# African-Robotics-Unit/AcinoSet

Hardware: AMD Instinct MI355X
Metric: FTE frames/sec (residual+Jac+LM step), 6-cam x 20-joint (higher is better)
Workload: dtype f64

## Files before the change

acinoset_amd/csrc/chunk.hip:

```cpp
#include "chunk.hpp"

#include <algorithm>
#include <cstdlib>
#include <type_traits>

#include "bcr_dev.hpp"
#include "trio80.hpp"

namespace acino {

void ChunkPlan::build(int nodes_total, int chunk_nodes, bool pin_l, bool pin_r) {
  n_nodes = nodes_total;
  m = n_chunks = n_sep = 0;
  node0 = pin_l ? 1 : 0;
  pin_right = pin_r ? 1 : 0;
  const int nodes = nodes_total - node0;
  if (chunk_nodes < 0 || nodes < 1) return;
  int mm = chunk_nodes;
  if (mm == 0) {
    mm = (nodes + 255) / 256;
    mm = std::max(4, std::min(mm, 512));
  }
  mm = std::max(2, mm);
  m = mm;
  n_chunks = (nodes + mm - 1) / mm;
  if (pin_r && n_chunks > 1 && nodes - (n_chunks - 1) * mm == 1) --n_chunks;
  n_sep = n_chunks - 1 + node0 + pin_right;
}

__device__ __forceinline__ void tile_store(double* M, int ib, int jb, const d4& a, int li, int lk) {
#pragma unroll
  for (int rr = 0; rr < 4; ++rr) M[(ib * 16 + lk + 4 * rr) * LD + jb * 16 + li] = a[rr];
}

constexpr int SW_VEC = 18 * NP + 2 * BS + 8 + 8 + 3 * NP + 64;
static constexpr size_t kSweepLds = (3 * MAT + SW_VEC) * sizeof(double);

__device__ __forceinline__ int opaque(int x) {
  asm volatile("" : "+v"(x));
  return x;
}

__device__ __forceinline__ unsigned opaque_u(unsigned x) {
  asm volatile("" : "+v"(x));
  return x;
}
struct BuildSlot {
  int pr, pc, base, e;
  bool own, dg;
  static __device__ __forceinline__ BuildSlot unpack(unsigned w) {
    BuildSlot s;
    s.pr = w & 31;
    s.pc = (w >> 5) & 31;
    s.own = (w >> 10) & 1;
    s.dg = (w >> 11) & 1;
    s.base = (w >> 12) & 2047;
    s.e = w >> 23;
    return s;
  }
};
static_assert((NP - 1) * LD + NP - 1 < 2048 && 13 * NP <= 512 && NP <= 32, "BuildSlot's bit fields");

constexpr int SW_T = 512;
template <int NQ>
__device__ __forceinline__ void syrk_mask_n(d4 (&acc)[NQ], bool load) {
#pragma unroll
  for (int q = 0; q < NQ; ++q)
#pragma unroll
    for (int rr = 0; rr < 4; ++rr) acc[q][rr] = load ? acc[q][rr] : 0.0;
}
constexpr int SP_STEPS = 4 * NT - 1;
__device__ __forceinline__ void spike_gf(const double* G, const double (&bF)[NT][4], d4 (&acc)[NT], int li, int lk) {
  double a[3][NT];
  const double* gb = G + lk * LD + li;
  auto fetch = [&](int buf, int step) {
#pragma unroll
    for (int ib = 0; ib < NT; ++ib) a[buf][ib] = gb[(4 * step) * LD + ib * 16];
  };
#pragma unroll
  for (int ib = 0; ib < NT; ++ib) acc[ib] = d4{0, 0, 0, 0};
  fetch(0, 0);
  fetch(1, 1);
#pragma unroll
  for (int step = 0; step < SP_STEPS; ++step) {
    if (step + 2 < SP_STEPS) fetch((step + 2) % 3, step + 2);
    __builtin_amdgcn_sched_barrier(0);
#pragma unroll
    for (int ib = 0; ib < NT; ++ib) acc[ib] = mfma(a[step % 3][ib], bF[step >> 2][step & 3], acc[ib]);
    __builtin_amdgcn_sched_barrier(0);
  }
}
template <int NQ>
__device__ __forceinline__ void spike_ftt(d4 (&acc)[NQ], const double* Yf, const d4 (&T)[NT], const int (&as)[NQ], int li, int lk) {
  constexpr int DEPTH = NQ >= 3 ? 2 : (NQ == 2 ? 3 : 6);
  const double* p = Yf + lk * LD + li;
  double a[DEPTH + 1][NQ];
#pragma unroll
  for (int d = 0; d < DEPTH; ++d)
#pragma unroll
    for (int q = 0; q < NQ; ++q) a[d][q] = p[(4 * d) * LD + as[q] * 16];
#pragma unroll
  for (int st = 0; st < SP_STEPS; ++st) {
    if (st + DEPTH < SP_STEPS) {
#pragma unroll
      for (int q = 0; q < NQ; ++q) a[(st + DEPTH) % (DEPTH + 1)][q] = p[(4 * (st + DEPTH)) * LD + as[q] * 16];
    }
    __builtin_amdgcn_sched_barrier(0);
#pragma unroll
    for (int q = 0; q < NQ; ++q) acc[q] = mfma(-a[st % (DEPTH + 1)][q], T[st >> 2][st & 3], acc[q]);
    __builtin_amdgcn_sched_barrier(0);
  }
}
template <int NQ>
struct AlTiles {
  d4 acc[NQ];
  int as[NQ], j;
  double* Ag;
  __device__ __forceinline__ double* at(int q, int rr, int li, int lk) const {
    return as[q] >= j ? Ag + (size_t)(as[q] * 16 + 4 * rr + lk) * BS + j * 16 + li
                      : Ag + (size_t)(j * 16 + li) * BS + as[q] * 16 + 4 * rr + lk;
  }
  __device__ __forceinline__ void fetch(int li, int lk) {
#pragma unroll
    for (int q = 0; q < NQ; ++q)
#pragma unroll
      for (int rr = 0; rr < 4; ++rr) acc[q][rr] = *at(q, rr, li, lk);
  }
  __device__ __forceinline__ void run(bool load, const double* Yf, const d4 (&T)[NT], int li, int lk) {
    syrk_mask_n<NQ>(acc, load);
    spike_ftt<NQ>(acc, Yf, T, as, li, lk);
#pragma unroll
    for (int q = 0; q < NQ; ++q)
#pragma unroll
      for (int rr = 0; rr < 4; ++rr) *at(q, rr, li, lk) = acc[q][rr];
  }
};
__device__ __forceinline__ int role8(int wave) { return (0x75236410u >> (4 * wave)) & 15; }
constexpr int ctri_i(int t) { return (t >= 1) + (t >= 3) + (t >= 6) + (t >= 10); }
template <int T>
struct GramTile {
  static constexpr int ib = ctri_i(T), jb = T - ib * (ib + 1) / 2, ns = 4 * (NT - ib);
};
template <int T>
__device__ __forceinline__ void gram_fetch(const double* X, int li, int lk, double (&a)[GramTile<T>::ns], double (&b)[GramTile<T>::ns]) {
  const double* pa = X + (GramTile<T>::ib * 16 + li) * LD + GramTile<T>::ib * 16 + lk;
  const double* pb = X + (GramTile<T>::jb * 16 + li) * LD + GramTile<T>::ib * 16 + lk;
#pragma unroll
  for (int s = 0; s < GramTile<T>::ns; ++s) {
    a[s] = pa[4 * s];
    b[s] = pb[4 * s];
  }
}
template <int T>
__device__ __forceinline__ void gram_tile(double* Xg, int li, int lk, const double (&a)[GramTile<T>::ns], const double (&b)[GramTile<T>::ns]) {
  constexpr int ib = GramTile<T>::ib, jb = GramTile<T>::jb;
  d4 g = {0, 0, 0, 0};
#pragma unroll
  for (int s = 0; s < GramTile<T>::ns; ++s) g = mfma(a[s], b[s], g);
#pragma unroll
  for (int rr = 0; rr < 4; ++rr) {
    Xg[(ib * 16 + lk + 4 * rr) * LD + jb * 16 + li] = g[rr];
    if (ib != jb) Xg[(jb * 16 + li) * LD + ib * 16 + lk + 4 * rr] = g[rr];
  }
}
template <int T0, int... REST>
__device__ __forceinline__ void gram_chain(const double* Xf, double* Xg, int li, int lk, const double (&a)[GramTile<T0>::ns],
                                           const double (&b)[GramTile<T0>::ns]) {
  if constexpr (sizeof...(REST) > 0) {
    constexpr int rest[] = {REST...};
    double an[GramTile<rest[0]>::ns], bn[GramTile<rest[0]>::ns];
    gram_fetch<rest[0]>(Xf, li, lk, an, bn);
    __builtin_amdgcn_sched_barrier(0);
    gram_tile<T0>(Xg, li, lk, a, b);
    __builtin_amdgcn_sched_barrier(0);
    gram_chain<REST...>(Xf, Xg, li, lk, an, bn);
  } else {
    gram_tile<T0>(Xg, li, lk, a, b);
  }
}
template <int T0, int... REST>
__device__ __forceinline__ void gram_fixed(const double* Xf, double* Xg, int* done, int li, int lk, int lane) {
  double a[GramTile<T0>::ns], b[GramTile<T0>::ns];
  gram_fetch<T0>(Xf, li, lk, a, b);
  gram_chain<T0, REST...>(Xf, Xg, li, lk, a, b);
  asm volatile("" ::: "memory");
  if (lane == 0) __hip_atomic_fetch_add(done, 1 + (int)sizeof...(REST), __ATOMIC_RELAXED, __HIP_MEMORY_SCOPE_WORKGROUP);
  asm volatile("" ::: "memory");
}

struct SpikeArgs {
  const double* Xg;
  double* Y;
  double* Ag;
  const double* cRk;
  const double* bvn;
  double* zk;
  int *c_gfdone, *c_fready, *c_bv, *tdone;
  int *g_open, *g_done;
  const double* Xf;
  int k, n_s;
  bool hasL, has_next;
  long long* stamps;
};
template <int ROLE>
__device__ __forceinline__ void spike_node(const SpikeArgs& A, int& tsb, int ln) {
  constexpr bool two = ROLE == 5;
  constexpr int j0 = ROLE == 4 ? 1 : (ROLE == 5 ? 2 : (ROLE == 6 ? 3 : 4));
  constexpr int NA = ROLE == 4 ? 3 : (ROLE == 5 ? 2 : (ROLE == 6 ? 5 : 4));
  const int li = ln & 15, lk = ln >> 4;
  double* const Y = A.Y;
  auto stamp = [&](int i) { if (A.stamps && ln == 0) A.stamps[i] = (long long)wall_clock64(); };
  AlTiles<NA> al;
  AlTiles<1> al0;
  al.Ag = A.Ag;
  al.j = j0;
  if (ROLE == 4) { al.as[0] = 1; al.as[1] = 0; al.as[2 % NA] = 2; }
  if (ROLE == 5) { al.as[0] = 2; al.as[1] = 0; }
  if (ROLE == 6) { al.as[0] = 3; al.as[1] = 0; al.as[2 % NA] = 1; al.as[3 % NA] = 2; al.as[4 % NA] = 4; }
  if (ROLE == 7) { al.as[0] = 4; al.as[1] = 0; al.as[2 % NA] = 1; al.as[3 % NA] = 2; }
  al0.Ag = A.Ag;
  al0.j = 0;
  al0.as[0] = 0;
  if (A.hasL) {
    al.fetch(li, lk);
    if (two) al0.fetch(li, lk);
  }
  if (ROLE >= 6) {
    double* const Xg = const_cast<double*>(A.Xg);
    lds_wait(A.g_open, A.k + 1);
    if (ROLE == 6) gram_fixed<2, 13>(A.Xf, Xg, A.g_done, li, lk, ln);
    else if (A.hasL) gram_fixed<5, 9, 14>(A.Xf, Xg, A.g_done, li, lk, ln);
    else gram_fixed<2, 5, 9, 13, 14>(A.Xf, Xg, A.g_done, li, lk, ln);
  }
  lds_wait(A.g_done, 15 * (A.k + 1));
  stamp(16 + 4 * (ROLE - 4));
  d4 T0[NT], T1[NT];
  {
    double bF[NT][4];
    const double* yb = Y + lk * LD + j0 * 16 + li;
#pragma unroll
    for (int kb = 0; kb < NT; ++kb)
#pragma unroll
      for (int s = 0; s < 4; ++s) bF[kb][s] = (4 * kb + s < SP_STEPS) ? yb[(kb * 16 + 4 * s) * LD] : 0.0;
    spike_gf(A.Xg, bF, T0, li, lk);
  }
  if (two) {
    double bF[NT][4];
    const double* yb = Y + lk * LD + li;
#pragma unroll
    for (int kb = 0; kb < NT; ++kb)
#pragma unroll
      for (int s = 0; s < 4; ++s) bF[kb][s] = (4 * kb + s < SP_STEPS) ? yb[(kb * 16 + 4 * s) * LD] : 0.0;
    spike_gf(A.Xg, bF, T1, li, lk);
  }
  lds_signal(A.c_gfdone, ln);
  stamp(17 + 4 * (ROLE - 4));
  if (A.hasL) {
    lds_wait(A.c_fready, A.n_s * A.k);
    al.run(A.k > 0, Y, T0, li, lk);
    if (two) al0.run(A.k > 0, Y, T1, li, lk);
  }
  stamp(18 + 4 * (ROLE - 4));
  if (A.hasL) {
    if (ROLE != 5) lds_signal(A.tdone + (ROLE == 4 ? 0 : (ROLE == 6 ? 1 : 2)), ln);
    if (ROLE == 7 || ROLE == 4 || ROLE == 5) lds_wait(A.tdone + 1, A.k + 1);
    if (ROLE == 4 || ROLE == 5) lds_wait(A.tdone + 2, A.k + 1);
    if (ROLE == 5) lds_wait(A.tdone + 0, A.k + 1);
  }
  (void)tsb;
#pragma unroll
  for (int ib = 0; ib < NT; ++ib) tile_store(Y, ib, j0, T0[ib], li, lk);
  if (two) {
#pragma unroll
    for (int ib = 0; ib < NT; ++ib) tile_store(Y, ib, 0, T1[ib], li, lk);
  }
  if (ROLE == 7) {
    A.zk[ln] = Y[ln * LD + (BS - 1)];
    if (ln < 16) A.zk[64 + ln] = Y[(64 + ln) * LD + (BS - 1)];
  }
  if (A.has_next) {
    lds_wait(A.c_bv, A.k + 1);
    const double* const cRk = A.cRk;
    const double* const bvn = A.bvn;
    const int p = ln % NP, cg = ln / NP;
#pragma unroll
    for (int h = 0; h < (two ? 2 : 1); ++h) {
      const int c_lo = 16 * (h ? 0 : j0);
      if (cg < 2) {
        const double e00 = cRk[(0 * 3 + 0) * NP + p], e01 = cRk[(0 * 3 + 1) * NP + p], e02 = cRk[(0 * 3 + 2) * NP + p];
        const double e11 = cRk[(1 * 3 + 1) * NP + p], e12 = cRk[(1 * 3 + 2) * NP + p], e22 = cRk[(2 * 3 + 2) * NP + p];
        const double b0 = bvn[p], b1 = bvn[NP + p], b2 = bvn[2 * NP + p];
        double fv[8][3];
#pragma unroll
        for (int q = 0; q < 8; ++q) {
          const int cc = c_lo + cg + 2 * q;
          fv[q][0] = Y[p * LD + cc];
          fv[q][1] = Y[(NP + p) * LD + cc];
          fv[q][2] = Y[(2 * NP + p) * LD + cc];
        }
#pragma unroll
        for (int q = 0; q < 8; ++q) {
          const int cc = c_lo + cg + 2 * q;
          const double f0 = fv[q][0], f1 = fv[q][1], f2 = fv[q][2];
          double o0 = -(e00 * f0 + e01 * f1 + e02 * f2), o1 = -(e11 * f1 + e12 * f2), o2 = -(e22 * f2);
          if (cc == BS - 1) {
            o0 += b0;
            o1 += b1;
            o2 += b2;
          }
          Y[p * LD + cc] = o0;
          Y[(NP + p) * LD + cc] = o1;
          Y[(2 * NP + p) * LD + cc] = o2;
        }
      }
      if (ln < 16)
        for (int r = 3 * NP; r < BS; ++r) Y[r * LD + c_lo + ln] = 0.0;
    }
  }
  lds_signal(A.c_fready, ln);
  stamp(19 + 4 * (ROLE - 4));
}


__global__ void __launch_bounds__(SW_T)
k_chunk_sweep(BcrChain ch, SepView sp, const FteConst* __restrict__ cst, int* numeric_err, const int* __restrict__ status,
                int m, int n_chunks, int node0, int pin_right) {
  extern __shared__ __attribute__((aligned(16))) char smem_raw[];
  if (status && *status != 0) return;
  double* const Xf = reinterpret_cast<double*>(smem_raw);
  double* const Xg = Xf + MAT;
  double* const Y = Xg + MAT;
  double* const cL = Y + MAT;
  double* const cR0 = cL + 9 * NP;
  double* const bvb = cR0 + 9 * NP;
  double* const red = bvb + 2 * BS;
  int* const sync = reinterpret_cast<int*>(red + 8);
  int* const cB = sync + 5;
  int* const tdone = sync + 2;
  int* const g_done = sync + 6;
  int* const g_open = sync + 10;
  int* const c_gfdone = sync + 7;
  int* const c_fready = sync + 8;
  int* const c_bv = sync + 9;
  double* const kq = red + 16;
  double* const klo = kq + NP;
  double* const khi = klo + NP;
  long long* const lst = reinterpret_cast<long long*>(khi + NP);
  const int tid = threadIdx.x, wave = tid >> 6, lane = tid & 63;
  const FteConst& K = *cst;
  const int c = blockIdx.x;
  const int first = node0 + c * m;
  const bool hasL = c > 0 || node0 > 0, hasR = c + 1 < n_chunks || pin_right;
  const int len = c + 1 < n_chunks ? m : ch.n_nodes - first;
  const int n_int = hasR ? len - 1 : len;
  const int sL = c - 1 + node0, sR = c + node0;
  const size_t MB = (size_t)BS * BS;
  const int role = __builtin_amdgcn_readfirstlane(role8(wave));
  const bool uni_tables = coupling_tables_uniform(K, first, first + n_int - 1);
  const int n_s = hasL ? 4 : 1;
  const bool builder = role <= 3;
  const bool strips = role >= 4 && (hasL || role == 7);
  double gmax_run = 0.0;
  long long* const dbgp = (ch.dbg && (long long)blockIdx.x == ch.dbg[64] && ch.dbg[66] == 0) ? ch.dbg : nullptr;
  const int dbg_k = dbgp ? (int)ch.dbg[65] : -1;
  if (dbgp && lane == 0) {
    const unsigned hw = __builtin_amdgcn_s_getreg((31 << 11) | 4);
    atomicOr(reinterpret_cast<unsigned long long*>(ch.dbg + 67), (unsigned long long)((hw >> 4) & 3) << (4 * wave));
    if (wave == 0) ch.dbg[68] = hw;
  }
#define SW_STAMP(i) do { if (dbgp && k == dbg_k && lane == 0) lst[i] = (long long)wall_clock64(); } while (0)
  if (tid < 16) sync[tid] = 0;
  if (tid < 64) lst[tid] = 0;
  if (dbgp && tid == 0) dbgp[70] = (long long)wall_clock64();
  if (c == 0 && node0) {
    for (int e = tid; e < BS * BS; e += SW_T) sp.D[e] = 0.0;
    if (tid < BS) sp.b[tid] = 0.0;
  }
  if (tid < NP) {
    kq[tid] = K.q_w[tid];
    klo[tid] = K.lo[tid];
    khi[tid] = K.hi[tid];
  }
  __syncthreads();

  TrioSync tsy;
  {
    NodeFetch f;
    build_fetch<SW_T>(f, ch, K, first, tid);
    fill_coupling_coef<SW_T>(cL, cR0, K, first, tid, kq);
    for (int e = tid; e < MAT; e += SW_T) Y[e] = 0.0;
    gmax_run = build_finish<SW_T>(Xf, bvb, f, K, first, tid, kq, klo, khi);
    __syncthreads();
    if (dbgp && tid == 0) lst[60] = (long long)wall_clock64();
    if (hasL)
      for (int e = tid; e < 9 * NP; e += SW_T) {
        const int pair = e / NP, p = e % NP, ii = pair / 3, jj = pair % 3;
        if (ii <= jj) Y[(ii * NP + p) * LD + jj * NP + p] = cL[e];
      }
    if (tid < BS) Y[tid * LD + (BS - 1)] = bvb[tid];
    __syncthreads();
    if (role < 3) chol80_trio(Xf, role, lane, numeric_err, sync, tsy);
    __syncthreads();
    if (dbgp && tid == 0) lst[61] = (long long)wall_clock64();
  }

  unsigned slot0 = 0, slot1 = 0;
  if (builder) {
    auto pack = [](int e, bool own, bool dg) {
      const int pa = e / 13, dd = e % 13, pc = pa + dd >= NP ? pa + dd - NP : pa + dd;
      return (unsigned)pa | (unsigned)pc << 5 | (unsigned)own << 10 | (unsigned)dg << 11 | (unsigned)(pa * LD + pc) << 12 | (unsigned)e << 23;
    };
    auto offdiag = [](int n) { return 13 * (n / 12) + 1 + n % 12; };
    const bool dg0 = role == 1 && lane < NP;
    const int n0 = role == 1 ? 192 + lane - NP : (role == 0 ? 0 : (role == 2 ? 64 : 128)) + lane;
    slot0 = pack(dg0 ? 13 * lane : offdiag(n0), true, dg0);
    const bool own1 = (role == 3 && lane < 35) || (role == 2 && lane < 34);
    slot1 = pack(own1 ? offdiag((role == 3 ? 231 : 266) + lane) : 0, own1, false);
  }
  int tb = 0, tsb = 0;
#pragma unroll 1
  for (int k = 0; k < n_int; ++k) {
    const int node = first + k, next = node + 1;
    const bool last = k + 1 == n_int;
    const bool has_next = !last || hasR;
    const int ln = opaque(lane);
    const int li = ln & 15, lk = ln >> 4;
    double* const cRk = (uni_tables || !(k & 1)) ? cR0 : cL;
    if (builder) {
      const int bw = role;
      const int bt = bw * 64 + ln;
      const int fb_next = 3 * (next - node0);
      const BuildSlot s0 = BuildSlot::unpack(opaque_u(slot0)), s1 = BuildSlot::unpack(opaque_u(slot1));
      const bool two = bw >= 2;
      double hq[2][3] = {{0, 0, 0}, {0, 0, 0}}, xq[3] = {0, 0, 0}, gq[3] = {0, 0, 0}, cvq[3] = {0, 0, 0}, lamq = 0.0;
      bool liveq[3] = {false, false, false}, ownq[3] = {false, false, false};
      if (has_next) {
        const int cur = ch.st->cur;
        const double* Hg = cur ? ch.H1 : ch.H0;
        lamq = ch.st->lam;
#pragma unroll
        for (int j = 0; j < 3; ++j)
          if (fb_next + j < K.n_frames) {
            hq[0][j] = Hg[(size_t)(fb_next + j) * HPAIRS + s0.e];
            if (two && s1.own) hq[1][j] = Hg[(size_t)(fb_next + j) * HPAIRS + s1.e];
          }
        if (s0.dg) {
          const int pdg = s0.pr;
          const double* xg = cur ? ch.x1 : ch.x0;
          const double* gg = cur ? ch.g1 : ch.g0;
#pragma unroll
          for (int j = 0; j < 3; ++j)
            if (fb_next + j < K.n_frames) {
              xq[j] = xg[(size_t)(fb_next + j + HALO) * NP + pdg];
              gq[j] = gg[(size_t)(fb_next + j) * NP + pdg];
            }
#pragma unroll
          for (int pr = 0; pr < 3; ++pr) {
            const int j = pr == 2 ? 1 : 0, jp = pr == 0 ? 1 : 2;
            if (fb_next + jp < K.n_frames)
              cvq[pr] = 2.0 * kq[pdg] * band_coef_clip(K.n_offset + fb_next + j, jp - j, K.n_global, K.clip_len);
          }
        }
#pragma unroll
        for (int j = 0; j < 3; ++j) {
          liveq[j] = fb_next + j < K.n_frames;
          ownq[j] = fb_next + j >= K.own_lo && fb_next + j < K.own_hi;
        }
      }
      if (bw == 0) SW_STAMP(0);
      lds_barrier(cB, tb, 4, ln);
      lds_wait(c_gfdone, n_s * k);
      if (bw == 0) SW_STAMP(1);
      if (bt == 0) __hip_atomic_fetch_add(g_open, 1, __ATOMIC_RELAXED, __HIP_MEMORY_SCOPE_WORKGROUP);
      if (k > 0 && !uni_tables) fill_coupling_coef<256>(nullptr, cRk, K, node, bt, kq);
      if (bw == 0) gram_fixed<0, 10>(Xf, Xg, g_done, li, lk, ln);
      else if (bw == 1) gram_fixed<1, 7>(Xf, Xg, g_done, li, lk, ln);
      else if (bw == 2) gram_fixed<4, 8, 12>(Xf, Xg, g_done, li, lk, ln);
      else gram_fixed<3, 6, 11>(Xf, Xg, g_done, li, lk, ln);
      SW_STAMP(32 + wave);
      lds_barrier(cB, tb, 4, ln);
      lds_wait(g_done, 15 * (k + 1));
      if (bw == 0) SW_STAMP(2);
#pragma unroll
      for (int j = 0; j < 3; ++j) asm volatile("" : "+v"(hq[0][j]), "+v"(hq[1][j]), "+v"(xq[j]), "+v"(gq[j]));
      asm volatile("" : "+v"(lamq));
      if (has_next) {
        double* const bvn = bvb + ((k + 1) & 1) * BS;
        double ca[2][6], cb[2][6], gv[2][3][3];
        auto slot_reads = [&](const BuildSlot& sl, double (&a)[6], double (&b)[6], double (&g)[3][3]) {
          const double *ta = cRk + sl.pr, *tb_ = cRk + sl.pc;
          a[0] = ta[0 * NP]; a[1] = ta[1 * NP]; a[2] = ta[2 * NP];
          a[3] = ta[4 * NP]; a[4] = ta[5 * NP]; a[5] = ta[8 * NP];
          b[0] = tb_[0 * NP]; b[1] = tb_[1 * NP]; b[2] = tb_[2 * NP];
          b[3] = tb_[4 * NP]; b[4] = tb_[5 * NP]; b[5] = tb_[8 * NP];
          const double* gp0 = Xg + sl.base;
#pragma unroll
          for (int jj = 0; jj < 3; ++jj) {
            const double* gp = gp0 + jj * NP * LD;
            g[jj][0] = gp[0];
            g[jj][1] = gp[NP];
            g[jj][2] = gp[2 * NP];
          }
        };
        auto slot_finish = [&](const BuildSlot& sl, auto may_diag, const double (&a)[6], const double (&b)[6], const double (&g)[3][3],
                               const double (&h)[3]) {
#pragma clang fp contract(off)
          constexpr bool DIAG = decltype(may_diag)::value;
          const int pr = sl.pr;
          const bool dg = DIAG && sl.dg;
          const double a00 = a[0], a01 = a[1], a02 = a[2], a11 = a[3], a12 = a[4], a22 = a[5];
          const double b00 = b[0], b01 = b[1], b02 = b[2], b11 = b[3], b12 = b[4], b22 = b[5];
          double mm[3][3], S[2][3];
#pragma unroll
          for (int jj = 0; jj < 3; ++jj) {
            const double g0 = g[jj][0], g1 = g[jj][1], g2 = g[jj][2];
            mm[jj][0] = __builtin_fma(g2, b02, __builtin_fma(g0, b00, g1 * b01));
            mm[jj][1] = __builtin_fma(g1, b11, g2 * b12);
            mm[jj][2] = g2 * b22;
          }
#pragma unroll
          for (int ii = 0; ii < 3; ++ii) {
            S[0][ii] = __builtin_fma(a02, mm[2][ii], __builtin_fma(a00, mm[0][ii], a01 * mm[1][ii]));
            S[1][ii] = __builtin_fma(a11, mm[1][ii], a12 * mm[2][ii]);
          }
          double v[3][3];
#pragma unroll
          for (int j = 0; j < 3; ++j)
#pragma unroll
            for (int jp = 0; jp < 3; ++jp) v[j][jp] = (j == jp ? h[j] : 0.0);
          if (dg) {
#pragma unroll
            for (int j = 0; j < 3; ++j) {
              double d = 1.0, bb = 0.0;
              if (liveq[j]) {
                d = h[j];
                const double gtol = GRAD_ZERO_REL * d;
                const bool fixed = (xq[j] <= klo[pr] && gq[j] > gtol) || (xq[j] >= khi[pr] && gq[j] < -gtol);
                d = __builtin_fma(lamq, fmax(d, DIAG_FLOOR), d);
                if (fixed) d *= FIX_SCALE;
                bb = fixed ? 0.0 : -gq[j];
                if (ownq[j]) gmax_run = fmax(gmax_run, fabs(bb));
              }
              v[j][j] = d;
              bvn[j * NP + pr] = bb;
            }
            v[0][1] = v[1][0] = cvq[0];
            v[0][2] = v[2][0] = cvq[1];
            v[1][2] = v[2][1] = cvq[2];
          }
          double val[3][3];
#pragma unroll
          for (int jp = 0; jp < 3; ++jp) {
            val[0][jp] = v[0][jp] - S[0][jp];
            val[1][jp] = v[1][jp] - S[1][jp];
          }
          val[2][0] = __builtin_fma(-a22, mm[2][0], v[2][0]);
          val[2][1] = v[2][1] - a22 * mm[2][1];
          val[2][2] = __builtin_fma(-a22, mm[2][2], v[2][2]);
          if (sl.own) {
            double* const xa = Xf + sl.base;
            double* const xt = Xf + sl.pc * LD + pr;
#pragma unroll
            for (int j = 0; j < 3; ++j)
#pragma unroll
              for (int jp = 0; jp < 3; ++jp) {
                xa[j * NP * LD + jp * NP] = val[j][jp];
                if (!dg) xt[jp * NP * LD + j * NP] = val[j][jp];
              }
          }
        };
        const BuildSlot b0 = BuildSlot::unpack(opaque_u(slot0)), b1 = BuildSlot::unpack(opaque_u(slot1));
        slot_reads(b0, ca[0], cb[0], gv[0]);
        slot_finish(b0, std::true_type{}, ca[0], cb[0], gv[0], hq[0]);
        if (two) {
          slot_reads(b1, ca[1], cb[1], gv[1]);
          slot_finish(b1, std::false_type{}, ca[1], cb[1], gv[1], hq[1]);
        }
        if (bt < BS - 3 * NP) {
          Xf[(3 * NP + bt) * LD + 3 * NP + bt] = 1.0;
          bvn[3 * NP + bt] = 0.0;
        }
      }
      lds_barrier(cB, tb, 4, ln);
      if (bt == 0) __hip_atomic_fetch_add(c_bv, 1, __ATOMIC_RELAXED, __HIP_MEMORY_SCOPE_WORKGROUP);
      if (bw == 0) SW_STAMP(4);
      if (bw < 3) {
        if (!last) chol80_trio<false>(Xf, bw, ln, numeric_err, sync, tsy, (dbgp && k == dbg_k) ? lst : nullptr);
        SW_STAMP(8 + wave);
      } else if (bw == 3) {
        double* Gg = ch.D + node * MB;
#pragma unroll 6
        for (int q = 0; q < LOWER_ITEMS / 64; ++q) {
          const int idx = ln + 64 * q;
          int r, cc;
          lower_item(idx, r, cc);
          *reinterpret_cast<double2*>(Gg + r * BS + cc) = make_double2(Xg[r * LD + cc], Xg[r * LD + cc + 1]);
        }
        SW_STAMP(8 + wave);
      }
    }
    if (strips) {
      SpikeArgs sa;
      sa.Xg = Xg; sa.Y = Y; sa.Ag = sp.AL + (size_t)(hasL ? opaque(sL) : 0) * MB; sa.cRk = cRk; sa.bvn = bvb + ((k + 1) & 1) * BS;
      sa.zk = ch.b + (size_t)node * BS; sa.g_open = g_open; sa.g_done = g_done; sa.Xf = Xf; sa.c_gfdone = c_gfdone; sa.c_fready = c_fready; sa.c_bv = c_bv; sa.tdone = tdone;
      sa.k = k; sa.n_s = n_s; sa.hasL = hasL; sa.has_next = has_next; sa.stamps = (dbgp && k == dbg_k) ? lst : nullptr;
      if (role == 4) spike_node<4>(sa, tsb, ln);
      else if (role == 5) spike_node<5>(sa, tsb, ln);
      else if (role == 6) spike_node<6>(sa, tsb, ln);
      else spike_node<7>(sa, tsb, ln);
    }
  }
  __syncthreads();
  if (dbgp) {
    if (tid == 0) lst[62] = (long long)wall_clock64();
    __syncthreads();
    if (tid < 64 && lst[tid]) dbgp[tid] = lst[tid];
  }
  if (hasR) {
    {
      double2* d2 = reinterpret_cast<double2*>(sp.D + (size_t)sR * MB);
      for (int idx = tid; idx < BS * BS / 2; idx += SW_T) {
        const int e = 2 * idx, r = e / BS, cc = e % BS;
        d2[idx] = make_double2(Xf[r * LD + cc], Xf[r * LD + cc + 1]);
      }
    }
    if (tid < BS) sp.b[(size_t)sR * BS + tid] = Y[tid * LD + (BS - 1)];
    if (hasL) {
      double* Cg = sp.Cpl + (size_t)sL * MB;
      for (int e = tid; e < BS * BS; e += SW_T) {
        const int r = e / BS, cc = e % BS;
        Cg[e] = cc < 3 * NP ? Y[r * LD + cc] : 0.0;
      }
    }
  }
#undef SW_STAMP
  publish_gmax<SW_T>(gmax_run, red, ch.gn_part, c, tid);
  if (dbgp && tid == 0) dbgp[71] = (long long)wall_clock64();
}

__global__ void __launch_bounds__(256) k_sep_combine(SepView sp, const int* __restrict__ status) {
  if (status && *status != 0) return;
  const int q = blockIdx.x, tid = threadIdx.x;
  const size_t MB = (size_t)BS * BS;
  double* D = sp.D + q * MB;
  const double* A = sp.AL + q * MB;
  constexpr int NQ = (LOWER_ITEMS + 255) / 256;
  double2 dv[NQ], av[NQ];
  const double bq = tid < 3 * NP ? sp.b[(size_t)q * BS + tid] : 0.0, aq = tid < 3 * NP ? A[(size_t)(BS - 1) * BS + tid] : 0.0;
#pragma unroll
  for (int k = 0; k < NQ; ++k) {
    const int idx = tid + 256 * k;
    if (idx < LOWER_ITEMS) {
      int r, cc;
      lower_item(idx, r, cc);
      dv[k] = *reinterpret_cast<const double2*>(D + r * BS + cc);
      av[k] = *reinterpret_cast<const double2*>(A + r * BS + cc);
    }
  }
#pragma unroll
  for (int k = 0; k < NQ; ++k) {
    const int idx = tid + 256 * k;
    if (idx < LOWER_ITEMS) {
      int r, cc;
      lower_item(idx, r, cc);
      if (r < 3 * NP) {
        const double ax = cc < 3 * NP ? av[k].x : 0.0, ay = cc + 1 < 3 * NP ? av[k].y : 0.0;
        *reinterpret_cast<double2*>(D + r * BS + cc) = make_double2(dv[k].x + ax, dv[k].y + ay);
      }
    }
  }
  if (tid < 3 * NP) sp.b[(size_t)q * BS + tid] = bq + aq;
}

constexpr int BK_PW = 4;
constexpr int BK_NL = 4;
constexpr int BK_T = 64 * (BK_PW + BK_NL);
constexpr int BK_NB = 2;
constexpr int BLD = 82;
constexpr int BK_Q = LOWER_ITEMS / 64;
constexpr int BK_FL = 8;
static_assert(LOWER_ITEMS == 64 * NT * (NT + 1), "30 rounds of 64 items: 2 (ib + 1) per tile row");
static_assert(BK_FL >= BK_NL + BK_NB + 2, "a far f_k must have been stored (and waited for) before a loader asks for it");
constexpr int BK_OPS = BS * BLD, BK_TAB = BK_OPS + 5 * BS, BK_STAGE = BK_TAB + 9 * NP + 1;
static constexpr size_t kBacksubLds =
    (BK_NB * BK_STAGE + 2 * BS + BK_FL * BS + 2 * 9 * NP + 16 + NP + 1) * sizeof(double) + 16 * sizeof(int);

typedef double d2 __attribute__((ext_vector_type(2)));
template <int CTRL>
__device__ __forceinline__ double dpp_add(double v) {
  const long long b = __double_as_longlong(v);
  const int lo = __builtin_amdgcn_update_dpp(0, (int)b, CTRL, 0xf, 0xf, false);
  const int hi = __builtin_amdgcn_update_dpp(0, (int)(b >> 32), CTRL, 0xf, 0xf, false);
  return v + __longlong_as_double(((long long)hi << 32) | (unsigned)lo);
}
__device__ __forceinline__ double lanes8_sum(double v) {
  v = dpp_add<0x141>(v);
  v = dpp_add<0xB1>(v);
  return dpp_add<0x4E>(v);
}
__global__ void __launch_bounds__(BK_T)
k_chunk_backsub(BcrChain ch, SepView sp, const FteConst* __restrict__ cst, const int* __restrict__ status, int m,
                int n_chunks, int node0, int pin_right, TrialOut trial) {
  extern __shared__ __attribute__((aligned(16))) char smem_raw[];
  double* const stg = reinterpret_cast<double*>(smem_raw);
  double* const ub = stg + BK_NB * BK_STAGE;
  double* const fl = ub + 2 * BS;
  double* const cL0 = fl + BK_FL * BS;
  double* const cRl = cL0 + 9 * NP;
  double* const red = cRl + 9 * NP;
  double* const kq = red + 16;
  int* const sync = reinterpret_cast<int*>(kq + NP + 1);
  int* const c_ready = sync;
  int* const c_rd = sync + BK_NL;
  int* const c_u = sync + BK_NL + 1;
  const int tid = threadIdx.x, lane = tid & 63, wave = tid >> 6;
  const int c = blockIdx.x, first = node0 + c * m;
  const bool hasL = c > 0 || node0 > 0, hasR = c + 1 < n_chunks || pin_right;
  const int len = c + 1 < n_chunks ? m : ch.n_nodes - first;
  const int n_int = hasR ? len - 1 : len;
  const int sL = c - 1 + node0, sR = c + node0;
  const size_t MB = (size_t)BS * BS;
  const int nf = hasL && n_int > 0 ? n_int - 1 : 0;
  const int ns = nf + n_int;
  auto node_at = [&](int s) __attribute__((always_inline)) { return s < nf ? s : n_int - 1 - (s - nf); };
  struct Rounds {
    int row0[BK_Q], col0[BK_Q];
    constexpr Rounds() : row0{}, col0{} {
      int q = 0;
      for (int ib = 0; ib < NT; ++ib)
        for (int h = 0; h < 2; ++h)
          for (int jc = 0; jc <= ib; ++jc) {
            row0[q] = 16 * ib + 8 * h;
            col0[q] = 16 * jc;
            ++q;
          }
    }
  };
  constexpr Rounds RD{};
  const int gl = (lane >> 3) * BS + 2 * (lane & 7), ll = (lane >> 3) * BLD + 2 * (lane & 7);
  d2 g[BK_Q];
  const int gl74 = ((lane >> 3) < 3 ? (lane >> 3) : 2) * BS + 2 * (lane & 7);
  auto tile_fetch = [&](int k) __attribute__((always_inline)) {
    const double* G = ch.D + (size_t)(first + k) * MB;
#pragma unroll
    for (int q = 0; q < BK_Q; ++q)
      g[q] = *reinterpret_cast<const d2*>(G + (RD.row0[q] * BS + RD.col0[q]) + (RD.row0[q] + 8 > 3 * NP ? gl74 : gl));
  };
  const int lw = wave - BK_PW;
  if (lw >= 0 && lw < ns) tile_fetch(node_at(lw));
  if (status && *status != 0) return;
  const FteConst& K = *cst;
  const bool uni = coupling_tables_uniform(K, first, first + n_int - 1);
  auto table_node = [&](int s) __attribute__((always_inline)) {
    const int k = node_at(s);
    return s < nf ? k : (k > 0 ? k - 1 : 0);
  };
  const int t_cur = ch.st->cur, t_nf = K.n_frames;
  const double* t_x = t_cur ? ch.x1 : ch.x0;
  const double* t_g = t_cur ? ch.g1 : ch.g0;
  const double* t_hd = t_cur ? trial.hd1 : trial.hd0;
  double* const fst = ch.Wl + (size_t)first * BS;
  if (ch.dbg && (long long)blockIdx.x == ch.dbg[64] && ch.dbg[66] == 1 && tid == 0) ch.dbg[61] = (long long)wall_clock64();
  if (c == 0 && sp.flags) {
    for (int e = tid; e < sp.n_flags; e += BK_T) sp.flags[e] = 0;
    if (tid == 0) sp.flags[sp.n_flags] += 1;
  }
  if (tid < 16) sync[tid] = 0;
  if (tid < 2 * BS) ub[tid] = 0.0;
  if (tid < NP) kq[tid] = K.q_w[tid];
  fill_coupling_coef<BK_T>(cL0, nullptr, K, first, tid);
  fill_coupling_coef<BK_T>(nullptr, cRl, K, first + (n_int > 0 ? n_int - 1 : 0), tid);
  double t_pred = 0.0, t_step = 0.0;
  if (wave >= BK_PW) {
    constexpr int NRO = (5 * 3 * NP + 63) / 64;
    double ro[NRO];
    auto ro_fetch = [&](int t) __attribute__((always_inline)) {
      if (t < nf) return;
      const int k = node_at(t), node = first + k;
      const bool far = hasL && k >= 1 && n_int - k >= BK_FL;
      const int ln = opaque(lane);
#pragma unroll
      for (int j = 0; j < NRO; ++j) {
        const int e = ln + 64 * j < 5 * 3 * NP ? ln + 64 * j : 5 * 3 * NP - 1, o = e / (3 * NP), r = e % (3 * NP);
        int n = 3 * (node - node0) + r / NP;
        n = n < t_nf ? n : t_nf - 1;
        const size_t nr = (size_t)n * NP + r % NP;
        const double* src = o == 0 ? ch.b + (size_t)node * BS + r
                          : o == 1 ? t_x + nr + (size_t)HALO * NP
                          : o == 2 ? t_g + nr
                          : o == 3 ? t_hd + nr
                                   : fst + (size_t)(far ? k - 1 : 0) * BS + r;
        ro[j] = *src;
      }
      if (lane < BS - 3 * NP) ch.b[(size_t)node * BS + 3 * NP + lane] = 0.0;
    };
    if (lw < ns) ro_fetch(lw);
    __syncthreads();
    for (int t = lw; t < ns; t += BK_NL) {
      const bool bwd = t >= nf;
      long long* const ldbg = (ch.dbg && (long long)blockIdx.x == ch.dbg[64] && ch.dbg[66] == 1 && lane == 0 && t >= 10 && t < 14) ? ch.dbg + 48 + 4 * (t - 10) : nullptr;
      if (ldbg) ldbg[0] = (long long)wall_clock64();
      if (t >= BK_NB) lds_wait(c_rd, BK_PW * (t - BK_NB + 1));
      if (ldbg) { __builtin_amdgcn_s_waitcnt(0x0F70); ldbg[1] = (long long)wall_clock64(); }
      double* const St = stg + (t % BK_NB) * BK_STAGE;
#pragma unroll
      for (int q = 0; q < BK_Q; ++q) *reinterpret_cast<d2*>(St + ll + (RD.row0[q] * BLD + RD.col0[q])) = g[q];
      if (bwd) {
        const int ln = opaque(lane);
#pragma unroll
        for (int j = 0; j < NRO; ++j) {
          const int e = ln + 64 * j;
          if (e < 5 * 3 * NP) St[BK_OPS + (e / (3 * NP)) * BS + e % (3 * NP)] = ro[j];
        }
      }
      if (uni) {
        if (t < BK_NB) right_table_interior<64>(St + BK_TAB, lane, [&](int p) { return kq[p]; });
      } else if (right_table_is_interior(K, first + table_node(t))) {
        right_table_interior<64>(St + BK_TAB, lane, [&](int p) { return kq[p]; });
      } else {
        fill_coupling_coef<64>(nullptr, St + BK_TAB, K, first + table_node(t), lane, kq);
      }
      if (ldbg) { __builtin_amdgcn_s_waitcnt(0xC07F); ldbg[2] = (long long)wall_clock64(); }
      lds_signal(c_ready + lw, lane);
      if (t + BK_NL < ns) {
        tile_fetch(node_at(t + BK_NL));
        ro_fetch(t + BK_NL);
      }
    }
  } else {
    const int pg = lane >> 3, part = lane & 7;
    const int p = 8 * wave + pg, pc = p < NP ? p : NP - 1;
    const int a = part < 3 ? part : 2, ra = a * NP + pc;
    const bool rowl = p < NP && part < 3;
    const int t_own_lo = K.own_lo, t_own_hi = K.own_hi;
    const double t_lam = ch.st->lam;
    double* t_xt = const_cast<double*>(t_cur ? ch.x0 : ch.x1);
    const double t_lo = K.lo[pc], t_hi = K.hi[pc];
    auto trial_row = [&](int node, double delta, double xv, double gv, double d0) __attribute__((always_inline)) {
      const int n = 3 * (node - node0) + a;
      if (rowl && n < t_nf) {
        const double gtol = GRAD_ZERO_REL * d0;
        const bool fixed = (xv <= t_lo && gv > gtol) || (xv >= t_hi && gv < -gtol);
        const double d = fixed ? 0.0 : delta, pg_ = fixed ? 0.0 : gv;
        const double xnew = fmin(fmax(xv + d, t_lo), t_hi);
        t_xt[(size_t)(n + HALO) * NP + pc] = xnew;
        if (n >= t_own_lo && n < t_own_hi) {
          t_pred += 0.5 * d * (t_lam * fmax(d0, DIAG_FLOOR) * d - pg_);
          t_step = fmax(t_step, fabs(xnew - xv));
        }
      }
    };
    constexpr int NJ = BS / 8;
    int gdir[3], gtrn[3], gtile[3];
#pragma unroll
    for (int aa = 0; aa < 3; ++aa) {
      const int r = aa * NP + pc;
      gdir[aa] = r * BLD + part;
      gtrn[aa] = part * BLD + r;
      gtile[aa] = r >> 4;
    }
    double xr[3] = {0, 0, 0}, xl[3] = {0, 0, 0};
    if (hasR) {
#pragma unroll
      for (int ii = 0; ii < 3; ++ii) xr[ii] = sp.b[(size_t)sR * BS + ii * NP + pc];
      if (tid < BS) ch.b[(size_t)(first + n_int) * BS + tid] = sp.b[(size_t)sR * BS + tid];
    }
    if (hasL) {
#pragma unroll
      for (int jj = 0; jj < 3; ++jj) xl[jj] = sp.b[(size_t)sL * BS + jj * NP + pc];
    }
    double s_xv, s_gv, s_d0;
    {
      int n = 3 * (first + n_int - node0) + a;
      n = n < t_nf ? n : t_nf - 1;
      s_xv = t_x[(size_t)(n + HALO) * NP + pc];
      s_gv = t_g[(size_t)n * NP + pc];
      s_d0 = t_hd[(size_t)n * NP + pc];
    }
    __syncthreads();
    double wR = 0.0, f0 = 0.0;
#pragma unroll
    for (int ii = 0; ii < 3; ++ii)
      if (ii <= a) wR += cRl[(ii * 3 + a) * NP + pc] * xr[ii];
#pragma unroll
    for (int jj = 0; jj < 3; ++jj)
      if (jj >= a) f0 += cL0[(a * 3 + jj) * NP + pc] * xl[jj];
    if (rowl) {
      ub[ra] = nf > 0 ? f0 : f0 + wR;
      if (hasL) {
        fst[ra] = f0;
        fl[ra] = f0;
      }
    }
    lds_signal(c_u, lane);
    long long* const bdbg = (ch.dbg && (long long)blockIdx.x == ch.dbg[64] && ch.dbg[66] == 1 && tid == 0) ? ch.dbg : nullptr;
    if (bdbg) bdbg[62] = (long long)wall_clock64();
    double cf[6] = {0, 0, 0, 0, 0, 0};
    bool pend = false;
    int p_node = 0;
    double p_xa = 0.0, p_xv = 0.0, p_gv = 0.0, p_d0 = 0.0;
#pragma unroll 1
    for (int s = 0; s < ns; ++s) {
      const int b = s & 1;
      const bool fwd = s < nf;
      const int k = node_at(s), node = first + k;
      const double* const St = stg + (s % BK_NB) * BK_STAGE;
#define BK_STAMP(i) do { if (bdbg && s >= 8 && s < 16) { __builtin_amdgcn_s_waitcnt(0xC07F); bdbg[6 * (s - 8) + (i)] = (long long)wall_clock64(); } } while (0)
      lds_wait2(c_ready + (s % BK_NL), s / BK_NL + 1, c_u, BK_PW * (s + 1));
      BK_STAMP(0);
      BK_STAMP(1);
      double uv[NJ], gv[3][NJ];
#pragma unroll
      for (int j = 0; j < NJ; ++j) uv[j] = ub[b * BS + part + 8 * j];
#pragma unroll
      for (int aa = 0; aa < 3; ++aa) {
        const int gd = opaque(gdir[aa]), gt = opaque(gtrn[aa]);
#pragma unroll
        for (int j = 0; j < NJ; ++j) gv[aa][j] = St[(j >> 1) <= gtile[aa] ? gd + 8 * j : gt + 8 * j * BLD];
      }
      if (!uni || s < BK_NB) {
        const double* T = St + BK_TAB;
        cf[0] = T[0 * NP + pc]; cf[1] = T[1 * NP + pc]; cf[2] = T[2 * NP + pc];
        cf[3] = T[4 * NP + pc]; cf[4] = T[5 * NP + pc]; cf[5] = T[8 * NP + pc];
      }
      const double z0 = St[BK_OPS + pc], z1 = St[BK_OPS + NP + pc], z2 = St[BK_OPS + 2 * NP + pc];
      const double o_xv = St[BK_OPS + BS + ra], o_gv = St[BK_OPS + 2 * BS + ra], o_d0 = St[BK_OPS + 3 * BS + ra];
      const double o_f = St[BK_OPS + 4 * BS + ra];
      const double fnear = fl[((k > 0 ? k - 1 : 0) % BK_FL) * BS + ra];
      lds_signal(c_rd, lane);
      if (pend) {
        if (rowl) ch.b[(size_t)p_node * BS + ra] = p_xa;
        trial_row(p_node, p_xa, p_xv, p_gv, p_d0);
        pend = false;
      }
      BK_STAMP(2);
      double y[3];
#pragma unroll
      for (int aa = 0; aa < 3; ++aa) {
        double v0 = gv[aa][0] * uv[0], v1 = gv[aa][1] * uv[1];
#pragma unroll
        for (int j = 2; j < NJ; j += 2) {
          v0 = fma(gv[aa][j], uv[j], v0);
          v1 = fma(gv[aa][j + 1], uv[j + 1], v1);
        }
        y[aa] = lanes8_sum(v0 + v1);
      }
      if (bdbg && s >= 8 && s < 16) { asm volatile("" :: "v"(y[0]), "v"(y[1]), "v"(y[2])); bdbg[6 * (s - 8) + 3] = (long long)wall_clock64(); }
      if (fwd) {
        const double f0_ = -(cf[0] * y[0] + cf[1] * y[1] + cf[2] * y[2]);
        const double f1_ = -(cf[3] * y[1] + cf[4] * y[2]);
        const double f2_ = -(cf[5] * y[2]);
        const double fn = a == 0 ? f0_ : (a == 1 ? f1_ : f2_);
        if (rowl) {
          ub[(b ^ 1) * BS + ra] = s + 1 == nf ? fn + wR : fn;
          fl[((k + 1) % BK_FL) * BS + ra] = fn;
          fst[(size_t)(k + 1) * BS + ra] = fn;
        }
        if (s + 1 == nf) __builtin_amdgcn_s_waitcnt(0x0F70);
        lds_signal(c_u, lane);
        BK_STAMP(4);
      } else {
        const double x0 = z0 - y[0], x1 = z1 - y[1], x2 = z2 - y[2];
        const double xa = a == 0 ? x0 : (a == 1 ? x1 : x2);
        const double e0 = cf[0] * x0, e1 = cf[1] * x0 + cf[3] * x1, e2 = cf[2] * x0 + cf[4] * x1 + cf[5] * x2;
        const double fk = hasL ? (n_int - k < BK_FL ? fnear : o_f) : 0.0;
        if (rowl && k > 0) ub[(b ^ 1) * BS + ra] = fk + (a == 0 ? e0 : (a == 1 ? e1 : e2));
        lds_signal(c_u, lane);
        BK_STAMP(4);
        pend = true;
        p_node = node;
        p_xa = xa;
        p_xv = o_xv;
        p_gv = o_gv;
        p_d0 = o_d0;
      }
      if (bdbg && s >= 8 && s < 16) bdbg[6 * (s - 8) + 5] = (long long)wall_clock64();
    }
#undef BK_STAMP
    if (pend) {
      if (rowl) ch.b[(size_t)p_node * BS + ra] = p_xa;
      trial_row(p_node, p_xa, p_xv, p_gv, p_d0);
    }
    if (bdbg) bdbg[63] = (long long)wall_clock64();
    if (hasR) trial_row(first + n_int, a == 0 ? xr[0] : (a == 1 ? xr[1] : xr[2]), s_xv, s_gv, s_d0);
  }
  for (int off = 32; off > 0; off >>= 1) {
    t_pred += __shfl_down(t_pred, off, 64);
    t_step = fmax(t_step, __shfl_down(t_step, off, 64));
  }
  if (lane == 0 && wave < BK_PW) {
    red[2 * wave] = t_pred;
    red[2 * wave + 1] = t_step;
  }
  __syncthreads();
  if (tid == 0) {
    double sp_ = 0.0, sm = 0.0;
#pragma unroll
    for (int w = 0; w < BK_PW; ++w) {
      sp_ += red[2 * w];
      sm = fmax(sm, red[2 * w + 1]);
    }
    trial.pred_part[c] = sp_;
    trial.step_part[c] = sm;
  }
}

int chunk_set_func_attributes() {
  ACINO_HIP_CHECK(hipFuncSetAttribute(reinterpret_cast<const void*>(k_chunk_sweep),
                                      hipFuncAttributeMaxDynamicSharedMemorySize, (int)kSweepLds));
  ACINO_HIP_CHECK(hipFuncSetAttribute(reinterpret_cast<const void*>(k_chunk_backsub),
                                      hipFuncAttributeMaxDynamicSharedMemorySize, (int)kBacksubLds));
  return ACINO_OK;
}

int chunk_reduce(const BcrChain& ch, const ChunkPlan& pl, const SepView& sp, const BcrChain& sepch,
                 const BcrSchedule& sepsch, const FteConst* d_c, int* d_numeric_err, const int* d_status, hipStream_t s,
                 Profiler* prof) {
  {
    ProfSpan span(prof, PC_CHUNK_SWEEP, s, pl.n_nodes - pl.n_sep);
    hipLaunchKernelGGL(k_chunk_sweep, dim3(pl.n_chunks), dim3(SW_T), kSweepLds, s, ch, sp, d_c, d_numeric_err, d_status, pl.m,
                       pl.n_chunks, pl.node0, pl.pin_right);
  }
  ACINO_LAUNCH_CHECK();
  if (pl.n_sep == 0) return ACINO_OK;
  if (!sepsch.consumers_add_al) {
    {
      ProfSpan span(prof, PC_SEP_COMBINE, s, pl.n_sep);
      hipLaunchKernelGGL(k_sep_combine, dim3(pl.n_sep), dim3(256), 0, s, sp, d_status);
    }
    ACINO_LAUNCH_CHECK();
  }
  return bcr_reduce(sepch, sepsch, d_c, d_numeric_err, d_status, s, prof);
}

int chunk_backsub(const BcrChain& ch, const ChunkPlan& pl, const SepView& sp, const BcrChain& sepch,
                  const BcrSchedule& sepsch, const FteConst* d_c, int* d_numeric_err, const int* d_status, hipStream_t s,
                  Profiler* prof, const TrialOut& trial) {
  if (pl.n_sep > 0) {
    int rc = bcr_backsub(sepch, sepsch, d_c, d_status, s, prof, d_numeric_err);
    if (rc) return rc;
  }
  {
    ProfSpan span(prof, PC_CHUNK_BACKSUB, s, pl.n_nodes - pl.n_sep);
    hipLaunchKernelGGL(k_chunk_backsub, dim3(pl.n_chunks), dim3(BK_T), kBacksubLds, s, ch, sp, d_c, d_status, pl.m, pl.n_chunks, pl.node0,
                       pl.pin_right, trial);
  }
  ACINO_LAUNCH_CHECK();
  return ACINO_OK;
}

}
```

Baseline: 24.49 million.

## Hoist loop-invariant state to scalar regs and rebalance strip-0 stencil across spike waves

```diff
diff --git a/acinoset_amd/csrc/chunk.hip b/acinoset_amd/csrc/chunk.hip
--- a/acinoset_amd/csrc/chunk.hip
+++ b/acinoset_amd/csrc/chunk.hip
@@ -44,6 +44,15 @@
 __device__ __forceinline__ unsigned opaque_u(unsigned x) {
   asm volatile("" : "+v"(x));
   return x;
+}
+template <class T>
+__device__ __forceinline__ T run_const(T x) {
+  asm volatile("" : "+s"(x));
+  return x;
+}
+__device__ __forceinline__ double run_const(double x) {
+  const int lo = __builtin_amdgcn_readfirstlane(__double2loint(x)), hi = __builtin_amdgcn_readfirstlane(__double2hiint(x));
+  return __hiloint2double(run_const(hi), run_const(lo));
 }
 struct BuildSlot {
   int pr, pc, base, e;
@@ -197,6 +206,7 @@
   double* zk;
   int *c_gfdone, *c_fready, *c_bv, *tdone;
   int *g_open, *g_done;
+  int* c_t0;
   const double* Xf;
   int k, n_s;
   bool hasL, has_next;
@@ -247,6 +257,7 @@
   if (two) {
     double bF[NT][4];
     const double* yb = Y + lk * LD + li;
+    if (A.hasL) lds_wait(A.c_fready, A.n_s * A.k);
 #pragma unroll
     for (int kb = 0; kb < NT; ++kb)
 #pragma unroll
@@ -268,12 +279,13 @@
     if (ROLE == 5) lds_wait(A.tdone + 0, A.k + 1);
   }
   (void)tsb;
+  if (two) {
+#pragma unroll
+    for (int ib = 0; ib < NT; ++ib) tile_store(Y, ib, 0, T1[ib], li, lk);
+    lds_signal(A.c_t0, ln);
+  }
 #pragma unroll
   for (int ib = 0; ib < NT; ++ib) tile_store(Y, ib, j0, T0[ib], li, lk);
-  if (two) {
-#pragma unroll
-    for (int ib = 0; ib < NT; ++ib) tile_store(Y, ib, 0, T1[ib], li, lk);
-  }
   if (ROLE == 7) {
     A.zk[ln] = Y[ln * LD + (BS - 1)];
     if (ln < 16) A.zk[64 + ln] = Y[(64 + ln) * LD + (BS - 1)];
@@ -283,9 +295,8 @@
     const double* const cRk = A.cRk;
     const double* const bvn = A.bvn;
     const int p = ln % NP, cg = ln / NP;
-#pragma unroll
-    for (int h = 0; h < (two ? 2 : 1); ++h) {
-      const int c_lo = 16 * (h ? 0 : j0);
+    auto stencil = [&](auto strip) __attribute__((always_inline)) {
+      constexpr int c_lo = 16 * decltype(strip)::value;
       if (cg < 2) {
         const double e00 = cRk[(0 * 3 + 0) * NP + p], e01 = cRk[(0 * 3 + 1) * NP + p], e02 = cRk[(0 * 3 + 2) * NP + p];
         const double e11 = cRk[(1 * 3 + 1) * NP + p], e12 = cRk[(1 * 3 + 2) * NP + p], e22 = cRk[(2 * 3 + 2) * NP + p];
@@ -315,6 +326,11 @@
       }
       if (ln < 16)
         for (int r = 3 * NP; r < BS; ++r) Y[r * LD + c_lo + ln] = 0.0;
+    };
+    stencil(std::integral_constant<int, j0>{});
+    if (ROLE == 4) {
+      lds_wait(A.c_t0, A.k + 1);
+      stencil(std::integral_constant<int, 0>{});
     }
   }
   lds_signal(A.c_fready, ln);
@@ -339,6 +355,7 @@
   int* const tdone = sync + 2;
   int* const g_done = sync + 6;
   int* const g_open = sync + 10;
+  int* const c_t0 = sync + 1;
   int* const c_gfdone = sync + 7;
   int* const c_fready = sync + 8;
   int* const c_bv = sync + 9;
@@ -418,6 +435,23 @@
     slot1 = pack(own1 ? offdiag((role == 3 ? 231 : 266) + lane) : 0, own1, false);
   }
   int tb = 0, tsb = 0;
+  const int run_cur = run_const(__builtin_amdgcn_readfirstlane(ch.st->cur));
+  const double run_lam = run_const(ch.st->lam);
+  using GlobalIn = const double __attribute__((address_space(1)))*;
+  auto run_global = [](const double* p) { return reinterpret_cast<GlobalIn>(run_const(reinterpret_cast<uintptr_t>(p))); };
+  const GlobalIn Hg = run_global(run_cur ? ch.H1 : ch.H0);
+  const GlobalIn xg = run_global(run_cur ? ch.x1 : ch.x0);
+  const GlobalIn gg = run_global(run_cur ? ch.g1 : ch.g0);
+  const int n_frames = run_const(K.n_frames), own_lo = run_const(K.own_lo), own_hi = run_const(K.own_hi);
+  const int64_t n_offset = run_const(K.n_offset), n_global = run_const(K.n_global), clip_len = run_const(K.clip_len);
+  double bc_run[3] = {0.0, 0.0, 0.0};
+  if (uni_tables) {
+#pragma unroll
+    for (int pr = 0; pr < 3; ++pr) {
+      const int j = pr == 2 ? 1 : 0, jp = pr == 0 ? 1 : 2;
+      bc_run[pr] = run_const(band_coef_clip(n_offset + 3 * (first + 1 - node0) + j, jp - j, n_global, clip_len));
+    }
+  }
 #pragma unroll 1
   for (int k = 0; k < n_int; ++k) {
     const int node = first + k, next = node + 1;
@@ -425,6 +459,7 @@
     const bool has_next = !last || hasR;
     const int ln = opaque(lane);
     const int li = ln & 15, lk = ln >> 4;
+    if (role == 0) SW_STAMP(3);
     double* const cRk = (uni_tables || !(k & 1)) ? cR0 : cL;
     if (builder) {
       const int bw = role;
@@ -434,40 +469,38 @@
       const bool two = bw >= 2;
       double hq[2][3] = {{0, 0, 0}, {0, 0, 0}}, xq[3] = {0, 0, 0}, gq[3] = {0, 0, 0}, cvq[3] = {0, 0, 0}, lamq = 0.0;
       bool liveq[3] = {false, false, false}, ownq[3] = {false, false, false};
+      __builtin_amdgcn_s_waitcnt(0x0f70);
       if (has_next) {
-        const int cur = ch.st->cur;
-        const double* Hg = cur ? ch.H1 : ch.H0;
-        lamq = ch.st->lam;
+        lamq = run_lam;
 #pragma unroll
         for (int j = 0; j < 3; ++j)
-          if (fb_next + j < K.n_frames) {
+          if (fb_next + j < n_frames) {
             hq[0][j] = Hg[(size_t)(fb_next + j) * HPAIRS + s0.e];
             if (two && s1.own) hq[1][j] = Hg[(size_t)(fb_next + j) * HPAIRS + s1.e];
           }
         if (s0.dg) {
           const int pdg = s0.pr;
-          const double* xg = cur ? ch.x1 : ch.x0;
-          const double* gg = cur ? ch.g1 : ch.g0;
 #pragma unroll
           for (int j = 0; j < 3; ++j)
-            if (fb_next + j < K.n_frames) {
+            if (fb_next + j < n_frames) {
               xq[j] = xg[(size_t)(fb_next + j + HALO) * NP + pdg];
               gq[j] = gg[(size_t)(fb_next + j) * NP + pdg];
             }
 #pragma unroll
           for (int pr = 0; pr < 3; ++pr) {
             const int j = pr == 2 ? 1 : 0, jp = pr == 0 ? 1 : 2;
-            if (fb_next + jp < K.n_frames)
-              cvq[pr] = 2.0 * kq[pdg] * band_coef_clip(K.n_offset + fb_next + j, jp - j, K.n_global, K.clip_len);
+            if (fb_next + jp < n_frames)
+              cvq[pr] = 2.0 * kq[pdg] * (uni_tables ? bc_run[pr] : band_coef_clip(n_offset + fb_next + j, jp - j, n_global, clip_len));
           }
         }
 #pragma unroll
         for (int j = 0; j < 3; ++j) {
-          liveq[j] = fb_next + j < K.n_frames;
-          ownq[j] = fb_next + j >= K.own_lo && fb_next + j < K.own_hi;
+          liveq[j] = fb_next + j < n_frames;
+          ownq[j] = fb_next + j >= own_lo && fb_next + j < own_hi;
         }
       }
       if (bw == 0) SW_STAMP(0);
+      SW_STAMP(34 + (wave & 1) + 4 * (wave >> 2));
       lds_barrier(cB, tb, 4, ln);
       lds_wait(c_gfdone, n_s * k);
       if (bw == 0) SW_STAMP(1);
@@ -602,7 +635,7 @@
     if (strips) {
       SpikeArgs sa;
       sa.Xg = Xg; sa.Y = Y; sa.Ag = sp.AL + (size_t)(hasL ? opaque(sL) : 0) * MB; sa.cRk = cRk; sa.bvn = bvb + ((k + 1) & 1) * BS;
-      sa.zk = ch.b + (size_t)node * BS; sa.g_open = g_open; sa.g_done = g_done; sa.Xf = Xf; sa.c_gfdone = c_gfdone; sa.c_fready = c_fready; sa.c_bv = c_bv; sa.tdone = tdone;
+      sa.zk = ch.b + (size_t)node * BS; sa.g_open = g_open; sa.g_done = g_done; sa.Xf = Xf; sa.c_gfdone = c_gfdone; sa.c_fready = c_fready; sa.c_bv = c_bv; sa.tdone = tdone; sa.c_t0 = c_t0;
       sa.k = k; sa.n_s = n_s; sa.hasL = hasL; sa.has_next = has_next; sa.stamps = (dbgp && k == dbg_k) ? lst : nullptr;
       if (role == 4) spike_node<4>(sa, tsb, ln);
       else if (role == 5) spike_node<5>(sa, tsb, ln);
```

New measurement: 24.56 million (median of 6 runs). Within noise of the previous version (+0.3%).
